# Denizantip/py-numpy-renderer

Hardware: AMD Instinct MI355X
Metric: Mfrag/s (1920x1080, 200k tris + shadow volumes) (higher is better)
Workload: dtype f64; 1 GPU; torus 500x200 (200k tris) + floor, 1920x1080, point light, shadow volumes (BASELINE.json configs[3] / BASELINE.md c4); faces=200002, views=8, frames_in_flight=3, parallelism=screen tiles x1 (bands)

## Files before the change

include/mi355rast.h:

```cpp
#ifndef MI355RAST_H
#define MI355RAST_H

#include <stdint.h>

#ifdef __cplusplus
extern "C" {
#endif

#define MR_ABI_VERSION 4

enum {
    MR_OK = 0,
    MR_E_INVALID = -1,
    MR_E_DEVICE = -2,
    MR_E_UNSUPPORTED = -3,
    MR_E_OVERFLOW = -4
};

enum { MR_LIGHT_DIRECTIONAL = 0, MR_LIGHT_POINT = 1, MR_LIGHT_SPOT = 2 };

enum {
    MR_FACE_RENDERED = 0, MR_FACE_BACK_FACE_CULLING = 1, MR_FACE_WRONG_MIN_MAX = 2,
    MR_FACE_EMPTY_B = 4, MR_FACE_EMPTY_Z = 8, MR_FACE_CLIPPED = 16
};
// ... 137 lines not shown
void mr_host_camera_constants(const double *eye, const double *center, const double *up, const double *position,
                              const double *projection, int32_t lh, double *lookat, double *mvp, double *planes);

int mr_host_overlay_build(const double *corners, const double *planes, const double *mvp, const double *viewport,
                          double near_plane, double far_plane, int32_t camera_inside, int32_t height, int32_t width,
                          int32_t *n_segments, int32_t *n_points, int32_t *n_touched);
int mr_host_overlay_fetch(int32_t *seg_first, int32_t *seg_count, int32_t *target, int32_t *next, double *z,
                          int32_t *touched);

int mr_render_device(mr_scene *scene, const mr_frame_desc *frame, void *d_out_rgb, void *stream);

int mr_get_stats(mr_scene *scene, mr_stats *stats);

#define MR_N_KERNEL_TIMES 5
int mr_get_kernel_times(mr_scene *scene, int n_frames, float *out_ms, int cap);
int mr_get_stream_kernel_times(mr_scene *scene, void *stream, int n_frames, float *out_ms, int cap);

int mr_read_z(mr_scene *scene, double *out_hw);
int mr_read_stencil(mr_scene *scene, int16_t *out_hw);
int mr_read_winner(mr_scene *scene, int32_t *out_hw);
int mr_read_frame_f32(mr_scene *scene, float *out_hw3);
int mr_read_face_status(mr_scene *scene, uint8_t *out_faces);
int mr_read_silhouette(mr_scene *scene, int32_t *out_triples, int32_t cap);
int mr_read_stencil_light(mr_scene *scene, int32_t light, int16_t *out_hw);
int mr_read_silhouette_light(mr_scene *scene, int32_t light, int32_t *out_triples, int32_t cap);

#define MR_TILE_RECORD_WORDS 12
int mr_debug_read_tile_records(mr_scene *scene, uint32_t *out, int32_t cap_tiles);

int mr_debug_clusters_culled(mr_scene *scene);

int mr_debug_quad_walks(mr_scene *scene, uint32_t *out);

int mr_debug_force_full(mr_scene *scene, int32_t on);

int mr_debug_frame_path(mr_scene *scene, int32_t *out);

int mr_debug_sil_cache(mr_scene *scene, int32_t *out);

int mr_debug_read_tile_order(mr_scene *scene, uint32_t *out, int32_t cap_tiles);

int mr_scene_set_model_pose(mr_scene *scene, int32_t model, const double *m16);

int mr_scene_set_model_pose_normals(mr_scene *scene, int32_t model, const double *g9);

int mr_debug_pose(mr_scene *scene, int32_t *out);

#define MR_N_POSE_TIMES 5
int mr_debug_pose_times(mr_scene *scene, float *out_ms);

#define MR_N_POSE_NORMALS_TIMES 2
int mr_debug_pose_normals_times(mr_scene *scene, float *out_ms);

int mr_scene_set_model_skin(mr_scene *scene, int32_t model, const int32_t *joints, const double *weights, int32_t n_bones,
                            const int32_t *normal_owner);

int mr_scene_set_model_bones(mr_scene *scene, int32_t model, const double *bones16, int32_t n_bones);

void mr_host_skin_chain(const double *verts, const int32_t *joints, const double *weights, const double *bones, int32_t n, double *out);

void mr_host_skin_chain3(const double *vectors, const int32_t *owner, const int32_t *joints, const double *weights, const double *bones,
                         int32_t n, double *out);

int mr_debug_skin(mr_scene *scene, int32_t *out);

#define MR_N_SKIN_TIMES 2
// ... 34 lines not shown
```

py-numpy-renderer_amd/_native.py:

```python
import ctypes as C
import os
import zlib

import numpy as np

from ._pack import active_morph, active_skin, auto_normals_active, morph_csr, normal_owners, pack_frame, pack_model, pose_normal_matrix

_HERE = os.path.dirname(os.path.abspath(__file__))
LIB_NAME = "libmi355rast.so"
LIB_PATH = os.path.join(_HERE, LIB_NAME)

MR_OK = 0
MR_E_OVERFLOW = -4
FRAME_SHADOWS, FRAME_KEEP_FLOAT, FRAME_FACE_STATUS, FRAME_LIGHT_TIMING, FRAME_SKYBOX, FRAME_COUNTERS = 1, 2, 4, 8, 16, 32
FRAME_KEEP_BUFFERS = 64
FRAME_NO_TIMING = 128
FRAME_OVERLAY = 256
FRAME_SUPERSAMPLE2, FRAME_SUPERSAMPLE4 = 512, 1024
_SUPERSAMPLE_FLAGS = {1: 0, 2: FRAME_SUPERSAMPLE2, 4: FRAME_SUPERSAMPLE4}
ABI_VERSION = 4
MAX_LIGHTS = 4
TILE_RECORD_WORDS = 12


# ... 72 lines not shown
    "mr_scene_add_model": (C.c_int, [C.c_void_p, C.POINTER(ModelDesc)]),
    "mr_scene_clear": (C.c_int, [C.c_void_p]),
    "mr_scene_set_overlay": (C.c_int, [C.c_void_p, C.POINTER(OverlayDesc)]),
    "mr_scene_set_overlay_cameras": (C.c_int, [C.c_void_p, C.c_void_p, C.c_void_p, C.c_void_p, C.c_void_p, C.c_double, C.c_double,
                                               C.c_int32, C.c_int32, C.c_int32]),
    "mr_scene_set_list_capacities": (C.c_int, [C.c_void_p, C.c_uint32, C.c_uint32, C.c_uint32, C.c_uint32]),
    "mr_scene_set_extra_lights": (C.c_int, [C.c_void_p, C.c_void_p, C.c_int32]),
    "mr_read_stencil_light": (C.c_int, [C.c_void_p, C.c_int32, C.c_void_p]),
    "mr_read_silhouette_light": (C.c_int, [C.c_void_p, C.c_int32, C.c_void_p, C.c_int32]),
    "mr_render": (C.c_int, [C.c_void_p, C.POINTER(FrameDesc), C.c_void_p, C.POINTER(Stats)]),
    "mr_overlay_state_bytes": (C.c_int64, [C.c_void_p]),
    "mr_overlay_apply": (C.c_int, [C.c_void_p, C.c_void_p, C.c_int64, C.c_int64, C.c_int32, C.c_int32, C.c_int32, C.c_void_p, C.c_void_p]),
    "mr_render_async": (C.c_int, [C.c_void_p, C.POINTER(FrameDesc), C.c_void_p, C.c_int32]),
    "mr_render_wait": (C.c_int, [C.c_void_p, C.c_int32, C.POINTER(Stats)]),
    "mr_host_alloc": (C.c_void_p, [C.c_uint64]),
    "mr_host_free": (None, [C.c_void_p]),
    "mr_render_device": (C.c_int, [C.c_void_p, C.POINTER(FrameDesc), C.c_void_p, C.c_void_p]),
    "mr_get_stats": (C.c_int, [C.c_void_p, C.POINTER(Stats)]),
    "mr_get_kernel_times": (C.c_int, [C.c_void_p, C.c_int, C.POINTER(C.c_float), C.c_int]),
    "mr_get_stream_kernel_times": (C.c_int, [C.c_void_p, C.c_void_p, C.c_int, C.POINTER(C.c_float), C.c_int]),
    "mr_read_z": (C.c_int, [C.c_void_p, C.c_void_p]),
    "mr_read_stencil": (C.c_int, [C.c_void_p, C.c_void_p]),
    "mr_read_winner": (C.c_int, [C.c_void_p, C.c_void_p]),
    "mr_read_frame_f32": (C.c_int, [C.c_void_p, C.c_void_p]),
    "mr_read_face_status": (C.c_int, [C.c_void_p, C.c_void_p]),
    "mr_read_silhouette": (C.c_int, [C.c_void_p, C.c_void_p, C.c_int32]),
    "mr_host_matmul_chain": (None, [C.c_void_p, C.c_void_p, C.c_void_p, C.c_int32, C.c_int32, C.c_int32]),
    "mr_host_overlay_build": (C.c_int, [C.c_void_p, C.c_void_p, C.c_void_p, C.c_void_p, C.c_double, C.c_double, C.c_int32,
                                        C.c_int32, C.c_int32, C.c_void_p, C.c_void_p, C.c_void_p]),
    "mr_host_overlay_fetch": (C.c_int, [C.c_void_p, C.c_void_p, C.c_void_p, C.c_void_p, C.c_void_p, C.c_void_p]),
    "mr_debug_read_tile_records": (C.c_int, [C.c_void_p, C.c_void_p, C.c_int32]),
    "mr_debug_clusters_culled": (C.c_int, [C.c_void_p]),
    "mr_debug_quad_walks": (C.c_int, [C.c_void_p, C.c_void_p]),
    "mr_host_camera_constants": (None, [C.c_void_p] * 5 + [C.c_int32] + [C.c_void_p] * 3),
    "mr_debug_read_tile_order": (C.c_int, [C.c_void_p, C.c_void_p, C.c_int32]),
    "mr_debug_sil_cache": (C.c_int, [C.c_void_p, C.c_void_p]),
    "mr_debug_force_full": (C.c_int, [C.c_void_p, C.c_int32]),
    "mr_debug_frame_path": (C.c_int, [C.c_void_p, C.c_void_p]),
    "mr_scene_set_model_pose": (C.c_int, [C.c_void_p, C.c_int32, C.c_void_p]),
    "mr_scene_set_model_pose_normals": (C.c_int, [C.c_void_p, C.c_int32, C.c_void_p]),
    "mr_debug_pose_normals_times": (C.c_int, [C.c_void_p, C.POINTER(C.c_float)]),
    "mr_debug_pose": (C.c_int, [C.c_void_p, C.c_void_p]),
    "mr_debug_pose_times": (C.c_int, [C.c_void_p, C.POINTER(C.c_float)]),
    "mr_debug_read_clusters": (C.c_int, [C.c_void_p, C.c_void_p, C.c_int32]),
    "mr_scene_set_model_skin": (C.c_int, [C.c_void_p, C.c_int32, C.c_void_p, C.c_void_p, C.c_int32, C.c_void_p]),
    "mr_scene_set_model_bones": (C.c_int, [C.c_void_p, C.c_int32, C.c_void_p, C.c_int32]),
    "mr_host_skin_chain": (None, [C.c_void_p, C.c_void_p, C.c_void_p, C.c_void_p, C.c_int32, C.c_void_p]),
    "mr_host_skin_chain3": (None, [C.c_void_p, C.c_void_p, C.c_void_p, C.c_void_p, C.c_void_p, C.c_int32, C.c_void_p]),
    "mr_debug_skin": (C.c_int, [C.c_void_p, C.c_void_p]),
    "mr_debug_skin_times": (C.c_int, [C.c_void_p, C.POINTER(C.c_float)]),
    "mr_scene_set_model_morph": (C.c_int, [C.c_void_p, C.c_int32, C.c_int32] + [C.c_void_p] * 6),
    "mr_scene_set_model_morph_weights": (C.c_int, [C.c_void_p, C.c_int32, C.c_void_p, C.c_int32]),
    "mr_host_morph_chain": (C.c_int, [C.c_void_p, C.c_int32, C.c_int32, C.c_int32] + [C.c_void_p] * 5),
    "mr_debug_morph": (C.c_int, [C.c_void_p, C.c_void_p]),
    "mr_debug_morph_times": (C.c_int, [C.c_void_p, C.POINTER(C.c_float)]),
    "mr_scene_set_model_auto_normals": (C.c_int, [C.c_void_p, C.c_int32, C.c_int32]),
    "mr_host_auto_normals": (C.c_int, [C.c_void_p, C.c_int32, C.c_void_p, C.c_int32, C.c_void_p, C.c_int32, C.c_void_p]),
    "mr_debug_auto_normals": (C.c_int, [C.c_void_p, C.c_void_p]),
    "mr_debug_auto_normals_times": (C.c_int, [C.c_void_p, C.POINTER(C.c_float)]),
    "mr_last_error": (C.c_char_p, []),
}
EXPORTED_SYMBOLS = tuple(_PROTOTYPES)

_lib = None


# ... 489 lines not shown
        _check(fn(self.handle, out.ctypes.data), fn.__name__)
        return out

    def read_z(self):
        return self._tap(self.lib.mr_read_z, np.float64)

    def read_stencil(self, light=0):
        h, w = self._frame
        out = np.empty((h, w), dtype=np.int16)
        _check(self.lib.mr_read_stencil_light(self.handle, int(light), out.ctypes.data), "mr_read_stencil_light")
        return out

    def read_winner(self):
        return self._tap(self.lib.mr_read_winner, np.int32)

    def read_frame_f32(self):
        return self._tap(self.lib.mr_read_frame_f32, np.float32, (3,))

    def read_tile_records(self):
        n = _check(self.lib.mr_debug_read_tile_records(self.handle, (C.c_uint32 * TILE_RECORD_WORDS)(), 0),
                   "mr_debug_read_tile_records")
        out = np.empty((max(n, 1), TILE_RECORD_WORDS), dtype=np.uint32)
        _check(self.lib.mr_debug_read_tile_records(self.handle, out.ctypes.data, n), "mr_debug_read_tile_records")
        return out[:n]

    def clusters_culled(self):
        return int(_check(self.lib.mr_debug_clusters_culled(self.handle), "mr_debug_clusters_culled"))

    def quad_walks(self):
        out = (C.c_uint32 * 4)()
        _check(self.lib.mr_debug_quad_walks(self.handle, out), "mr_debug_quad_walks")
        return tuple(int(x) for x in out)

    def sil_cache(self):
        out = (C.c_int32 * 4)()
        _check(self.lib.mr_debug_sil_cache(self.handle, out), "mr_debug_sil_cache")
        return tuple(int(x) for x in out)

    def force_full(self, on=True):
        _check(self.lib.mr_debug_force_full(self.handle, 1 if on else 0), "mr_debug_force_full")

    def frame_path(self):
        out = (C.c_int32 * 5)()
        _check(self.lib.mr_debug_frame_path(self.handle, out), "mr_debug_frame_path")
        return dict(zip(("full", "split", "ss", "ml", "ordered"), (bool(x) for x in out)))

    def pose_counters(self):
        out = (C.c_int32 * 4)()
        _check(self.lib.mr_debug_pose(self.handle, out), "mr_debug_pose")
        return tuple(int(x) for x in out)

    def skin_counters(self):
        out = (C.c_int32 * 4)()
        _check(self.lib.mr_debug_skin(self.handle, out), "mr_debug_skin")
        return tuple(int(x) for x in out)

    def morph_counters(self):
        out = (C.c_int32 * 5)()
        _check(self.lib.mr_debug_morph(self.handle, out), "mr_debug_morph")
        return tuple(int(x) for x in out)

    def auto_normals_counters(self):
        out = (C.c_int32 * 4)()
        _check(self.lib.mr_debug_auto_normals(self.handle, out), "mr_debug_auto_normals")
        return tuple(int(x) for x in out)

# ... 72 lines not shown
```

py-numpy-renderer_amd/csrc/host_env.h:

```cpp
#pragma once

namespace {

struct Env {
    bool vertex_mfma, resolve_separate, sil_cache;
    int edge_spread, tile_split, tile_order;
    int quad_walk;
    unsigned split_cost, split_quads;
    const char *cluster_cull;
};

Env read_env()
{
    static const Env once = [] {
        auto is = [](const char *name, const char *value) { const char *e = getenv(name); return e && !strcmp(e, value); };
        auto number = [](const char *name, int unset) { const char *e = getenv(name); return e ? atoi(e) : unset; };
        Env e = {};
        e.vertex_mfma = is("MR_VERTEX_PATH", "mfma");
        e.resolve_separate = is("MR_RESOLVE_PATH", "separate");
        e.edge_spread = number("MR_EDGE_SPREAD", -2);
        e.tile_order = is("MR_TILE_ORDER", "rowmajor") ? 1 : is("MR_TILE_ORDER", "heaviest") ? 2 : 0;
        e.quad_walk = is("MR_QUAD_WALK", "strips") ? 1 : is("MR_QUAD_WALK", "spans") ? 2 : 0;
        e.tile_split = number("MR_TILE_SPLIT", -1);
        e.split_cost = (unsigned)number("MR_SPLIT_COST", 400);
        e.split_quads = (unsigned)number("MR_SPLIT_QUADS", 48);
        return e;
    }();
    Env e = once;
    e.cluster_cull = getenv("MR_CLUSTER_CULL");
    const char *sil = getenv("MR_SIL_CACHE");
    e.sil_cache = !(sil && !strcmp(sil, "0"));
    return e;
}

}
```

py-numpy-renderer_amd/csrc/host_frame.h:

```cpp
#pragma once

namespace {

constexpr int EVENT_RING = 512, N_MARKS = 6;

struct FrameSlot {
    hipStream_t stream = nullptr;
    int id = 0;
    DevBuf d_vout, d_vclip, d_tris, d_clips, d_status, d_count_list, d_quads, d_sil, d_counters;
    DevBuf d_bin_count, d_items[mr::BIN_CLASSES], d_work, d_tile_stats, d_hist, d_split;
    DevBuf d_z, d_winner, d_stencil, d_frame, d_out;
    DevBuf d_stencil_x[mr::MAX_LIGHTS - 1];
    static_assert(mr::MAX_LIGHTS == MR_MAX_LIGHTS, "the ABI's light count is the kernels'");
    int last_n_lights = 1;
    uint32_t bin_cap[mr::BIN_CLASSES] = { 0, 0, 0 }, work_cap = 0, quad_cap = 0;
    int bins_zeroed_for = 0;

    mr::Counters *h_counters = nullptr;
    mr::Sticky *h_sticky = nullptr;
    hipEvent_t ev_ring[EVENT_RING][N_MARKS] = {};
    uint8_t ev_marks[EVENT_RING] = {};
    hipEvent_t *ev = ev_ring[0];
    uint64_t frames_enqueued = 0;
    uint64_t last_serial = 0;
// ... 403 lines not shown
        { { k_setup<true, true>, k_setup<false, true> }, { k_setup<true, false>, k_setup<false, false> } },
        { { k_setup_full<true, true>, k_setup_full<false, true> }, { k_setup_full<true, false>, k_setup_full<false, false> } } };
    hipLaunchKernelGGL(kernel[p.full][!p.ml][!p.env.vertex_mfma], dim3(1 + p.face_blocks + edge_blocks), dim3(SETUP_BLOCK), 0, stream, ska);
    return ska.sil.mode == SIL_CAPTURE ? sc->sil.capture_launched(&sa.ctr->n_quads, stream) : MR_OK;
}

void launch_bin_work(FrameSlot *fs, const mr::FrameConst &fc, const FramePlan &p)
{
    using namespace mr;
    hipLaunchKernelGGL(k_bin_work, dim3(p.count_blocks + WORK_BLOCKS), dim3(256), 0, fs->stream, fc, bin_args(fs), fs->d_count_list.as<uint32_t>(),
                       fs->d_tris.as<TriRec>(), fs->d_clips.as<TriClip>(), fs->d_status.as<uint8_t>(), fs->ctr(fs->frames_enqueued), p.count_blocks);
}

int launch_tile(mr_scene *sc, FrameSlot *fs, const mr::FrameConst &fc, const FramePlan &p, const mr::FrameLights &lights, uint8_t *d_out)
{
    using namespace mr;
    TileKernArgs tka;
    tka.fc = fc;
    TileArgs &ta = tka.ta;
    ta.clips = fs->d_clips.as<TriClip>(); ta.quads = fs->d_quads.as<QuadRec>();
    ta.bin_count = fs->d_bin_count.as<uint32_t>();
    for (int c = 0; c < BIN_CLASSES; ++c) { ta.items[c] = fs->d_items[c].as<uint32_t>(); ta.cap[c] = fs->bin_cap[c]; }
    ta.tap_mask = (p.overlay && !p.taps_asked) ? fs->ov.list<uint8_t>(3) : nullptr;
    ta.zbuf = p.keep ? fs->d_z.as<double>() : nullptr;
    ta.winner = p.keep ? fs->d_winner.as<int32_t>() : nullptr;
    ta.stencil = p.keep ? fs->d_stencil.as<int32_t>() : nullptr;
    ta.tile_stats = fs->d_tile_stats.as<uint32_t>();
    ta.ctr = fs->ctr(fs->frames_enqueued); ta.next_ctr = fs->ctr(fs->frames_enqueued + 1); ta.sticky = fs->sticky();
    ta.order = p.ordered ? fs->d_hist.as<uint32_t>() : nullptr;
    ta.tile_class = reinterpret_cast<uint8_t *>(fs->d_hist.p) + p.order_bytes;
    ta.split_arrive = fs->d_split.as<uint32_t>(); ta.split_sten = fs->d_split.as<int32_t>() + HEAVY0_MAX;
    ta.split_cost = p.split_cost; ta.split_quads = p.split_quads; ta.split_max = p.split_max;
    ta.quad_walk = (uint32_t)p.env.quad_walk;
    ShadeArgs &sh = tka.sh;
    sh.tris = fs->d_tris.as<TriRec>(); sh.face_pos = sc->d_face_pos.p; sh.face_attr = sc->d_face_attr.as<FaceAttr>();
    sh.materials = sc->d_materials.as<Material>();
    sh.sky = sc->sky_size > 0 ? sc->d_sky.as<uint8_t>() : nullptr;
    sh.gamma_lut = sc->d_gamma.as<float>(); sh.out = d_out;
    sh.frame = (fc.flags & MR_FRAME_KEEP_FLOAT) ? fs->d_frame.as<float>() : nullptr;
    tka.ml.lights.n = 1;
    if (p.ml) tka.ml.lights = lights;
    for (int k = 1; p.ml && k < MAX_LIGHTS; ++k) tka.ml.stencil[k - 1] = p.keep && k < p.n_lights ? fs->d_stencil_x[k - 1].as<int32_t>() : nullptr;
    if (p.n_tiles <= 0) {
        HIP_TRY(hipMemsetAsync(ta.next_ctr, 0, sizeof(Counters), fs->stream));
        return MR_OK;
    }
    static const struct { void (*kernel)(const TileKernArgs); int front; } choice[2][6] = {
        { { k_tile<false, true, true>, 0 },            { k_tile<false, false, true>, 0 },
          { k_tile<true, true, false>, SPLIT_FRONT },  { k_tile<true, false, false>, SPLIT_FRONT },
          { k_tile<false, true, false>, 0 },           { k_tile<false, false, false>, 0 } },
        { { k_tile_full<false, true, true>, 0 },           { k_tile_full<false, false, true>, 0 },
          { k_tile_full<true, true, false>, SPLIT_FRONT }, { k_tile_full<true, false, false>, SPLIT_FRONT },
          { k_tile_full<false, true, false>, 0 },          { k_tile_full<false, false, false>, 0 } } };
    const auto &c = choice[p.full][(p.ml ? 0 : p.split ? 2 : 4) + !p.ss];
    hipLaunchKernelGGL(c.kernel, dim3((unsigned)(p.n_tiles + c.front)), dim3(TILE_PX), 0, fs->stream, tka);
    return MR_OK;
}

void launch_after_tile(mr_scene *sc, FrameSlot *fs, const mr_frame_desc *fr, const mr::FrameConst &fc, const FramePlan &p, uint8_t *d_out)
{
    using namespace mr;
    hipStream_t stream = fs->stream;
    if ((fc.flags & MR_FRAME_FACE_STATUS) && fc.n_faces > 0)
        hipLaunchKernelGGL(k_face_status, dim3(blocks_for(fc.n_faces, 256)), dim3(256), 0, stream, fc, fs->d_tris.as<TriRec>(),
                           fs->d_clips.as<TriClip>(), fs->d_z.as<double>(), fs->d_stencil.as<int32_t>(), fs->d_status.as<uint8_t>());
    if (p.overlay && p.partial) {
// ... 156 lines not shown
```

py-numpy-renderer_amd/csrc/kernels_tile.h:

```cpp
#pragma once

#include "kernels_bin.h"
#include "kernels_shade.h"

namespace mr {

__device__ __forceinline__ unsigned long long z_key(double z)
{
    const unsigned long long b = (unsigned long long)__double_as_longlong(z);
    return (b >> 63) ? ~b : (b | 0x8000000000000000ull);
}
__device__ __forceinline__ double z_unkey(unsigned long long k)
{
    const unsigned long long b = (k >> 63) ? (k & 0x7fffffffffffffffull) : ~k;
    return __longlong_as_double((long long)b);
}

template <bool MAYBE_SINGLE>
struct PairMath {
    double a0, a1, p0, p1, q0, q1, k0, k1, k2;
    float d00, d01, d11, inv_den;
    bool sbox, sz;
    __device__ __forceinline__ explicit PairMath(const TriRec &t)
    {
// ... 7 lines not shown
    }
    __device__ __forceinline__ void bary(double x, double y, float &u, float &v, float &w) const
    {
        const double r0 = (sbox ? x : y) - a0, r1 = (sbox ? y : x) - a1;
        const float d20 = (float)fma(r1, p1, r0 * p0);
        const float d21 = (float)fma(r1, q1, r0 * q0);
        v = (d11 * d20 - d01 * d21) * inv_den;
        w = (d00 * d21 - d01 * d20) * inv_den;
        u = 1.0f - v - w;
    }
    __device__ __forceinline__ void bary(int x, int y, float &u, float &v, float &w) const
    {
        bary((double)(sbox ? x : y), (double)(sbox ? y : x), true, u, v, w);
    }
    __device__ __forceinline__ double depth(float u, float v, float w) const
    {
        const float m0 = sz ? u : v, m1 = sz ? v : u;
        return fma((double)w, k2, fma((double)m1, k1, (double)m0 * k0));
    }
private:
    __device__ __forceinline__ void bary(double c0, double c1, bool, float &u, float &v, float &w) const
    {
        const double r0 = c0 - a0, r1 = c1 - a1;
        const float d20 = (float)fma(r1, p1, r0 * p0);
        const float d21 = (float)fma(r1, q1, r0 * q0);
        v = (d11 * d20 - d01 * d21) * inv_den;
        w = (d00 * d21 - d01 * d20) * inv_den;
        u = 1.0f - v - w;
    }
};

constexpr int SMALL_LANES = 4;

constexpr int SWEEP_CACHE_K = 2, SWEEP_CACHE_ROUNDS = 2;
struct SweepCache {
    unsigned long long key[SWEEP_CACHE_K];
    uint32_t meta;
};

struct TileBounds { int width, band_y0, band_y1; };

template <int SWEEP, bool FULL>
__device__ __forceinline__ void small_pair(const TileBounds &tb, const TriRec &t, int gx, int gy, bool rh,
                                           unsigned long long *s_key, int *s_win, int sub, int lanes, unsigned int &frags,
                                           SweepCache *cache = nullptr, int first = 0)
{
    const int x0 = max((int)t.x0, gx), x1 = min((int)t.x1, min(gx + TILE_W, tb.width));
    const int y0 = max(max((int)t.y0, gy), tb.band_y0), y1 = min(min((int)t.y1, gy + TILE_H), tb.band_y1);
    const PairMath<true> pm(t);
    const bool nodepth = FULL && ((t.flags >> 8) & FF_NO_DEPTH) != 0;
    const int bw = x1 - x0;
    if (cache) { cache->meta = 0; }
    if (bw <= 0) return;
    int px = x0 + sub, py = y0;
    while (px >= x1) { px -= bw; ++py; }
    int walked = 0;
    while (py < y1) {
        if (SWEEP == 0 || walked >= first) {
            float u, v, w;
            pm.bary(px, py, u, v, w);
            bool ok = u >= 0 && v >= 0 && w >= 0;
            if (FULL && ok && SWEEP == 0) ++frags;
            if (ok && (SWEEP == 1 || !nodepth)) {
                const double z = pm.depth(u, v, w);
                if (z == z) {
                    const int p = (py - gy) * TILE_W + (px - gx);
                    const unsigned long long k = z_key(z);
                    if (SWEEP == 0) {
                        if (rh) atomicMin(&s_key[p], k); else atomicMax(&s_key[p], k);
                        if (cache) {
#pragma unroll
                            for (int c = 0; c < SWEEP_CACHE_K; ++c)
                                if (walked == c) { cache->key[c] = k; cache->meta |= ((uint32_t)p << (8 * c)) | (1u << (16 + c)); }
                        }
                    } else if (nodepth ? (rh ? k <= s_key[p] : k >= s_key[p]) : s_key[p] == k) {
                        atomicMax(&s_win[p], t.face);
                    }
                }
            }
        }
        ++walked;
        px += lanes;
        while (px >= x1) { px -= bw; ++py; }
    }
    if (cache) cache->meta |= (uint32_t)walked << 20;
}

__device__ __forceinline__ int out_row(const FrameConst &fc, int py, int l)
{
    if (fc.out_tile_rows > 0)
        return (fc.out_tile_rows - 1 - l) * TILE_H + (tile_row_frame(fc, l) * TILE_H + TILE_H - 1 - py);
    return fc.band_y1 - 1 - py;
}

__device__ __forceinline__ uint8_t *ss_out_pixel(uint8_t *out, int width, int band_y1, int shift, int px, int py)
{
    return out + ((size_t)((band_y1 - 1 - py) >> shift) * (width >> shift) + (px >> shift)) * 3;
}
__device__ __forceinline__ void ss_block_mean(const float *rgb, int row, int shift, float m[3])
{
    const int s = 1 << shift;
    float acc[3] = { 0.f, 0.f, 0.f };
    for (int j = 0; j < s; ++j)
        for (int i = 0; i < s; ++i) {
#pragma unroll
            for (int c = 0; c < 3; ++c) acc[c] += rgb[j * row + i * 3 + c];
        }
    const float inv = 1.0f / (float)(s * s);
#pragma unroll
    for (int c = 0; c < 3; ++c) m[c] = acc[c] * inv;
}
__device__ __forceinline__ void ss_resolve_tile(const FrameConst &fc, const float *s_rgb, uint8_t *out, int gx, int gy, int tid,
                                                const float *s_gamma)
{
    const int shift = fc.ss_mode & SS_SHIFT_MASK, n_log = 4 - shift;
    static_assert(TILE_W == 16 && TILE_H == 16, "ss_resolve_tile");
    if (tid >= 1 << (2 * n_log)) return;
    const int bx = tid & ((1 << n_log) - 1), by = tid >> n_log;
// ... 55 lines not shown
#define MR_CLASS_SCALE 100
#endif
__device__ __forceinline__ int tile_class(uint32_t cost)
{
    const uint32_t c = cost * 100u / (uint32_t)MR_CLASS_SCALE;
    return c >= 500u ? 1 : c >= 350u ? 2 : c >= 250u ? 3 : c >= 170u ? 4 : c >= 110u ? 5 : c >= 70u ? 6 : c >= 40u ? 7 : 8;
}
static_assert(ORDER_CLASSES == 8, "tile_class");
#ifndef MR_HEAVY0_MAX
#define MR_HEAVY0_MAX 128
#endif
constexpr int HEAVY_SPLIT = 4, HEAVY0_MAX = MR_HEAVY0_MAX;
#ifndef MR_TILE_WAVES
#define MR_TILE_WAVES 5
#endif
constexpr int K_TILE_WAVES = MR_TILE_WAVES;
#ifndef MR_TILE_WAVES_1L
#define MR_TILE_WAVES_1L 6
#endif
constexpr int K_TILE_WAVES_1L = MR_TILE_WAVES_1L;
constexpr int SPLIT_FRONT = HEAVY_SPLIT * HEAVY0_MAX;

__device__ __forceinline__ uint32_t tile_cost(uint32_t n_small, uint32_t n_big, uint32_t n_quad)
{
    return 20u + 2u * n_small + 30u * n_big + 3u * n_quad;
}

struct TileArgs {
    const TriClip *clips;
    const QuadRec *quads;
    uint32_t *bin_count;
    const uint32_t *items[BIN_CLASSES];
    uint32_t cap[BIN_CLASSES];
    const uint8_t *tap_mask;
    double *zbuf;
    int32_t *winner, *stencil;
    uint32_t *tile_stats;
    Counters *ctr, *next_ctr;
    Sticky *sticky;
    int32_t *split_sten;
    uint32_t *split_arrive;
    const uint32_t *order;
    uint8_t *tile_class;
    uint32_t split_cost, split_quads;
    uint32_t split_max;
    uint32_t quad_walk;
};

struct TileLights {
    FrameLights lights;
    int32_t *stencil[MAX_LIGHTS - 1];
};
struct TileKernArgs { FrameConst fc; TileArgs ta; ShadeArgs sh; TileLights ml; };

template <bool SPLIT, bool SS, bool ML, bool FULL>
__device__ __forceinline__ void tile_body()
{
    static_assert(!(SPLIT && ML), "frames with several lights do not split their heavy tiles");
    __shared__ unsigned long long s_key[TILE_PX];
    __shared__ int s_win[TILE_PX];
    __shared__ unsigned int s_cnt[TILE_STATS];
    __shared__ uint4 s_quad[QUAD_BATCH * QUAD_STAGE_U4];
    __shared__ uint32_t s_id[QUAD_BATCH];
    __shared__ float s_gamma[GAMMA_LUT_SIZE];
    __shared__ unsigned long long s_mat[MAT_LDS * sizeof(Material) / 8];

// ... 77 lines not shown
                if (ss) {
                    float *s_rgb = reinterpret_cast<float *>(s_quad);
#pragma unroll
                    for (int j = 0; j < 3; ++j) s_rgb[lp * 3 + j] = rgb[j];
                }
                __syncthreads();
                if (ss) {
                    ss_resolve_tile(fc, reinterpret_cast<const float *>(s_quad), sh.out, gx, gy, tid, s_gamma);
                } else if (live) {
#pragma unroll
                    for (int j = 0; j < 3; ++j) o[j] = gamma_u8(rgb[j], s_gamma);
                }
            } else if (ss) {
                const int shift = ss & SS_SHIFT_MASK, n_log = 4 - shift;
                const int bpx = gx + ((tid & ((1 << n_log) - 1)) << shift), bpy = gy + ((tid >> n_log) << shift);
                if (tid < 1 << (2 * n_log) && bpx < fc.width && bpy >= fc.band_y0 && bpy < fc.band_y1) {
                    uint8_t *ob = ss_out_pixel(sh.out, fc.width, fc.band_y1, shift, bpx, bpy);
                    ob[0] = (uint8_t)fc.background_u8; ob[1] = (uint8_t)(fc.background_u8 >> 8); ob[2] = (uint8_t)(fc.background_u8 >> 16);
                }
            } else if (live) {
                o[0] = (uint8_t)fc.background_u8; o[1] = (uint8_t)(fc.background_u8 >> 8); o[2] = (uint8_t)(fc.background_u8 >> 16);
            }
            if (tid == 0) {
                uint32_t *rec = ta.tile_stats + (size_t)tile * TILE_REC;
                for (int k = 0; k < TILE_REC; ++k) rec[k] = 0;
                rec[7] = n_quad_raw;
                rec[8] = rec[10] = rec[11] = (uint32_t)t_start;
                rec[9] = (uint32_t)stamp();
                ta.bin_count[2 * n_tiles + tile] = 0;
                ta.tile_class[tile] = (uint8_t)ORDER_CLASSES;
            }
            return;
        }
        if (FULL && tid < TILE_STATS) s_cnt[tid] = 0;
        s_gamma[tid] = sh.gamma_lut[tid];
        if (tid == 0) s_gamma[GAMMA_LUT_SIZE - 1] = sh.gamma_lut[GAMMA_LUT_SIZE - 1];
        mat_lds = fc.n_materials <= MAT_LDS;
        if (mat_lds && tid < fc.n_materials * (int)(sizeof(Material) / 8))
            s_mat[tid] = reinterpret_cast<const unsigned long long *>(sh.materials)[tid];
    }
    auto my_pixel = [&](int &px, int &py) {
        int l = lp;
        asm volatile("" : "+v"(l));
        px = gx + (l & (TILE_W - 1)); py = gy + l / TILE_W;
    };

    double zbest = rh ? INFINITY : -INFINITY;
    int best = -1;
    {
        const TileKernArgs &ka = kernargs<TileKernArgs>();
        const FrameConst &fc = ka.fc;
        const TileArgs &ta = ka.ta;
        const ShadeArgs &sh = ka.sh;
        const TriRec *__restrict__ tris = sh.tris;
        const TriClip *__restrict__ clips = ta.clips;
        const uint32_t *__restrict__ small_items = ta.items[0] + (size_t)tile * ta.cap[0];
        const uint32_t *__restrict__ big_items = ta.items[1] + (size_t)tile * ta.cap[1];
        const bool same_clip = fc.same_clip != 0, has_no_depth = FULL && fc.has_no_depth != 0;
        const TileBounds tb = { fc.width, fc.band_y0, fc.band_y1 };
        int px, py;
        my_pixel(px, py);
        const double dpx = (double)px, dpy = (double)py;
        unsigned int frags = 0;
        constexpr int TRI_U4 = (int)(sizeof(TriRec) / 16);
        static_assert(WAVE * TRI_U4 <= QUAD_BATCH * QUAD_STAGE_U4, "big-pair records are staged in the quad area");
        auto big_pairs = [&](const bool late) {
// ... 17 lines not shown
                        float u, v, w;
                        pm.bary(dpx, dpy, u, v, w);
                        in = in && u >= 0 && v >= 0 && w >= 0;
                        const unsigned long long m = __ballot(in);
                        if (!m) return;
                        if (FULL && !late) frags += (unsigned int)__popcll(m);
                        if (nodepth && !late) return;
                        if (flags & TF_CLIP) {
                            if (in) {
                                const TriClip &c = clips[f];
                                double p[3];
                                persp_bary(t.dp, u, v, w, (flags & TF_SINGLE_BOX) != 0, p);
                                in = inside_clip(p, c.clip) && (same_clip || inside_clip(p, c.clipd));
                            }
                        }
                        const double z = pm.depth(u, v, w);
                        if (late) {
                            if (in && (rh ? z <= zbest : z >= zbest) && f > best) best = f;
                        } else {
                            const bool closer = rh ? (z < zbest) : (z > zbest);
                            if (in && (closer || (z == zbest && f > best))) { zbest = z; best = f; }
                        }
                    };
                    if (flags & (TF_SINGLE_BOX | TF_SINGLE_Z)) pair(std::true_type{});
                    else pair(std::false_type{});
                }
            }
        };
        big_pairs(false);
        if (n_small) { s_key[lp] = z_key(zbest); s_win[lp] = -1; }
        __syncthreads();
        if (FULL && lane == 0 && frags) atomicAdd(&s_cnt[0], frags);
        if (n_small) {
            unsigned long long (*c_key)[SWEEP_CACHE_K][TILE_PX] =
                reinterpret_cast<unsigned long long (*)[SWEEP_CACHE_K][TILE_PX]>(s_quad);
            uint32_t (*c_meta)[TILE_PX] = reinterpret_cast<uint32_t (*)[TILE_PX]>(
                reinterpret_cast<unsigned long long *>(s_quad) + SWEEP_CACHE_ROUNDS * SWEEP_CACHE_K * TILE_PX);
            uint32_t (*c_face)[TILE_PX] = c_meta + SWEEP_CACHE_ROUNDS;
            static_assert(SWEEP_CACHE_ROUNDS * TILE_PX * (SWEEP_CACHE_K * 8 + 8) <= (int)sizeof(s_quad), "sweep cache fits the quad area");
            unsigned int sfrags = 0;
            int round = 0;
            const int spl = n_small > (uint32_t)(TILE_PX / SMALL_LANES) ? SMALL_LANES / 2
                          : n_small > (uint32_t)(TILE_PX / (2 * SMALL_LANES)) ? SMALL_LANES : 2 * SMALL_LANES;
            const uint32_t per_round = (uint32_t)(TILE_PX / spl), my_pair = (uint32_t)(tid / spl);
            const int sub = tid % spl;
            for (uint32_t i = my_pair; i < n_small; i += per_round, ++round) {
                const TriRec t = tris[small_items[i]];
                if (round < SWEEP_CACHE_ROUNDS) {
                    SweepCache sc;
                    small_pair<0, FULL>(tb, t, gx, gy, rh, s_key, s_win, sub, spl, sfrags, &sc);
                    const bool nodepth = FULL && ((t.flags >> 8) & FF_NO_DEPTH) != 0;
#pragma unroll
                    for (int c = 0; c < SWEEP_CACHE_K; ++c) c_key[round][c][tid] = sc.key[c];
                    c_meta[round][tid] = nodepth ? (sc.meta & 0xfff00000u) : sc.meta;
                    c_face[round][tid] = (uint32_t)t.face | (nodepth ? 0x80000000u : 0u);
                } else {
                    small_pair<0, FULL>(tb, t, gx, gy, rh, s_key, s_win, sub, spl, sfrags);
                }
            }
            if (FULL && sfrags) atomicAdd(&s_cnt[0], sfrags);
            __syncthreads();

            const unsigned long long kfinal = s_key[lp];
            if (best >= 0 && kfinal == z_key(zbest)) atomicMax(&s_win[lp], best);
            round = 0;
            for (uint32_t i = my_pair; i < n_small; i += per_round, ++round) {
                int first = 0;
                if (round < SWEEP_CACHE_ROUNDS) {
                    const uint32_t meta = c_meta[round][tid], cf = c_face[round][tid];
                    const int walked = (int)(meta >> 20);
                    const bool nodepth = FULL && (cf >> 31) != 0;
#pragma unroll
                    for (int c = 0; c < SWEEP_CACHE_K; ++c)
                        if ((meta >> (16 + c)) & 1u) {
                            const int p = (int)((meta >> (8 * c)) & 0xffu);
                            if (s_key[p] == c_key[round][c][tid]) atomicMax(&s_win[p], (int)(cf & 0x7fffffffu));
                        }
                    if (!nodepth && walked <= SWEEP_CACHE_K) continue;
                    first = nodepth ? 0 : SWEEP_CACHE_K;
                }
                const TriRec t = tris[small_items[i]];
                small_pair<1, FULL>(tb, t, gx, gy, rh, s_key, s_win, sub, spl, sfrags, nullptr, first);
            }
            __syncthreads();
            best = s_win[lp];
            zbest = z_unkey(kfinal);
        }
        if (has_no_depth) big_pairs(true);
    }
    const bool covered = live && best >= 0;
    const unsigned long long t_raster = stamp();

    int sten = 0;
    int sten_x[MAX_LIGHTS - 1] = { 0, 0, 0 };
    unsigned int qfrags = 0, qupd = 0;
    if (n_quad && (counters || __syncthreads_or(covered))) {
        const TileKernArgs &ka = kernargs<TileKernArgs>();
        const FrameConst &fc = ka.fc;
        const TileArgs &ta = ka.ta;
        const uint32_t *__restrict__ quad_items = ta.items[2] + (size_t)tile * ta.cap[2];
        const QuadRec *__restrict__ quads = ta.quads;
        const double f_plus_n = fc.f_plus_n, f_minus_n = fc.f_minus_n, two_nf = fc.two_nf;
        double zlim = rh ? -INFINITY : INFINITY, zhard = rh ? INFINITY : -INFINITY;
        if (covered) zlim = zhard = zbest;
#pragma unroll
        for (int off = WAVE / 2; off; off >>= 1) {
            const double o = __shfl_xor(zlim, off), h = __shfl_xor(zhard, off);
            zlim = rh ? fmax(zlim, o) : fmin(zlim, o);
            zhard = rh ? fmin(zhard, h) : fmax(zhard, h);
        }
        if (!FULL) {
            zlim = __hiloint2double(__builtin_amdgcn_readfirstlane(__double2hiint(zlim)), __builtin_amdgcn_readfirstlane(__double2loint(zlim)));
            zhard = __hiloint2double(__builtin_amdgcn_readfirstlane(__double2hiint(zhard)), __builtin_amdgcn_readfirstlane(__double2loint(zhard)));
        }
        if (!ML && ta.quad_walk != QUAD_WALK_STRIPS) {
// ... 331 lines not shown
            ta.zbuf[at_px] = zbest;
            ta.winner[at_px] = best;
            ta.stencil[at_px] = sten;
        }
    }
    static_assert(TILE_PX * 3 * sizeof(float) <= sizeof(s_quad), "resolve staging fits the quad area");
    if (fused_ss) {
        __syncthreads();
        const TileKernArgs &ka = kernargs<TileKernArgs>();
        ss_resolve_tile(ka.fc, reinterpret_cast<const float *>(s_quad), ka.sh.out, gx, gy, tid, s_gamma);
    }

    if (counters) {
        const unsigned long long cov = __ballot(covered), litm = __ballot(covered && lit);
        if (ML) {
            unsigned int v = covered ? n_lit : 0u;
#pragma unroll
            for (int off = WAVE / 2; off; off >>= 1) v += (unsigned int)__shfl_xor((int)v, off);
            if (lane == 0 && v) atomicAdd(&s_cnt[4], v);
        }
        if (lane == 0) {
            if (cov) atomicAdd(&s_cnt[3], (unsigned int)__popcll(cov));
            if (!ML && litm) atomicAdd(&s_cnt[4], (unsigned int)__popcll(litm));
            if (qfrags) atomicAdd(&s_cnt[1], qfrags);
            if (qupd) atomicAdd(&s_cnt[2], qupd);
        }
    }
    if (FULL) __syncthreads();
    const TileArgs &ta = kernargs<TileKernArgs>().ta;
    uint32_t *rec = ta.tile_stats + (size_t)tile * TILE_REC;
    if (FULL && tid < TILE_STATS) rec[tid] = s_cnt[tid];
    if (tid == 0) {
        rec[5] = n_small_raw; rec[6] = n_big_raw; rec[7] = n_quad_raw;
        rec[8] = (uint32_t)t_start;
        rec[9] = (uint32_t)stamp();
        rec[10] = (uint32_t)t_raster; rec[11] = (uint32_t)t_quads;
        if (n_small_raw > ta.cap[0]) { atomicOr(&ta.ctr->overflow, 1u); atomicMax(&ta.ctr->max_list[0], n_small_raw); }
        if (n_big_raw > ta.cap[1]) { atomicOr(&ta.ctr->overflow, 2u); atomicMax(&ta.ctr->max_list[1], n_big_raw); }
        if (n_quad_raw > ta.cap[2]) { atomicOr(&ta.ctr->overflow, 4u); atomicMax(&ta.ctr->max_list[2], n_quad_raw); }
    }
    if (tid < BIN_CLASSES) ta.bin_count[tid * n_tiles + tile] = 0;
    if (tid == 0) {
        int cls = tile_class(cost);
        if (SPLIT) cls = (cost >= ta.split_cost && n_quad_raw >= ta.split_quads) ? 1 : cls < 2 ? 2 : cls;
        ta.tile_class[tile] = (uint8_t)cls;
    }
}

template <bool SPLIT, bool SS, bool ML>
__global__ void __launch_bounds__(TILE_PX, ML ? K_TILE_WAVES : K_TILE_WAVES_1L)
k_tile(const TileKernArgs)
{
    tile_body<SPLIT, SS, ML, false>();
}
template <bool SPLIT, bool SS, bool ML>
__global__ void __launch_bounds__(TILE_PX, ML ? K_TILE_WAVES : K_TILE_WAVES_1L)
k_tile_full(const TileKernArgs)
{
    tile_body<SPLIT, SS, ML, true>();
}

__global__ void __launch_bounds__(256)
k_reduce_tile_stats(const uint32_t *__restrict__ tile_stats, int n_tiles, Counters *__restrict__ ctr, int counted)
{
    constexpr int NS = TILE_STATS + 2;
    __shared__ unsigned long long part[NS][256 / WAVE];
    const int tid = threadIdx.x, lane = tid & (WAVE - 1), wv = tid / WAVE;
// ... 62 lines not shown
```

py-numpy-renderer_amd/csrc/mi355rast.hip:

```cpp
#include "../../include/mi355rast.h"
#include "host_overlay.h"

#include <hip/hip_runtime.h>

#include <algorithm>
#include <array>
#include <cmath>
#include <cstdio>
#include <cstdlib>
#include <cstring>
#include <memory>
#include <new>
#include <string>
#include <vector>

#include "rast_types.h"
#include "kernels_geometry.h"
#include "kernels_tile.h"
#include "kernels_overlay.h"
#include "kernels_pose.h"

#include "host_device.h"
#include "host_env.h"
#include "host_silcache.h"
// ... 757 lines not shown
    if (!out) return fail(MR_E_INVALID, "NULL argument");
    const int n = std::min(fs->last_n_tiles, cap_tiles);
    HIP_TRY(hipDeviceSynchronize());
    static_assert(mr::TILE_REC == MR_TILE_RECORD_WORDS, "tile record size is part of the ABI");
    if (n > 0) HIP_TRY(hipMemcpy(out, fs->d_tile_stats.p, (size_t)n * mr::TILE_REC * 4, hipMemcpyDeviceToHost));
    if (!fs->last_full)
        for (int t = 0; t < n; ++t)
            for (int k = 0; k < mr::TILE_STATS; ++k) out[(size_t)t * mr::TILE_REC + k] = 0u;
    return fs->last_n_tiles;
}

int mr_debug_clusters_culled(mr_scene *sc)
{
    FrameSlot *fs = last_slot(sc);
    if (!fs) return MR_E_INVALID;
    HIP_TRY(hipDeviceSynchronize());
    if (int rc = fetch_counters(fs, false)) return rc;
    HIP_TRY(hipStreamSynchronize(fs->stream));
    return (int)fs->h_counters->pad0[0];
}

int mr_debug_quad_walks(mr_scene *sc, uint32_t *out)
{
    FrameSlot *fs = last_slot(sc);
    if (!fs) return MR_E_INVALID;
    if (!out) return fail(MR_E_INVALID, "NULL argument");
    HIP_TRY(hipDeviceSynchronize());
    if (int rc = fetch_counters(fs, false)) return rc;
    HIP_TRY(hipStreamSynchronize(fs->stream));
    for (int k = 0; k < 4; ++k) out[k] = fs->h_counters->pad0[1 + k];
    return MR_OK;
}

int mr_debug_force_full(mr_scene *sc, int32_t on)
{
    if (!sc) return fail(MR_E_INVALID, "NULL argument");
    sc->force_full = on != 0;
    return MR_OK;
}

int mr_debug_frame_path(mr_scene *sc, int32_t *out)
{
    FrameSlot *fs = last_slot(sc);
    if (!fs) return MR_E_INVALID;
    if (!out) return fail(MR_E_INVALID, "NULL argument");
    out[0] = fs->last_full ? 1 : 0; out[1] = fs->last_split ? 1 : 0; out[2] = fs->last_ss_mode ? 1 : 0;
    out[3] = fs->last_n_lights > 1 ? 1 : 0; out[4] = fs->last_ordered ? 1 : 0;
    return MR_OK;
}

int mr_debug_sil_cache(mr_scene *sc, int32_t *out)
{
    if (!sc || !out) return fail(MR_E_INVALID, "NULL argument");
    out[0] = sc->sil.last_path; out[1] = (int32_t)sc->sil.last_entries; out[2] = (int32_t)sc->sil.captures;
    out[3] = sc->sil.valid_buffers();
    return MR_OK;
}

int mr_debug_pose(mr_scene *sc, int32_t *out)
{
    if (!sc || !out) return fail(MR_E_INVALID, "NULL argument");
    int32_t posed = 0;
    for (const mr_scene::ModelPose &mp : sc->poses) posed += mp.posed ? 1 : 0;
    out[0] = sc->commits; out[1] = sc->pose_passes; out[2] = posed; out[3] = sc->pose_written;
    return MR_OK;
}
// ... 132 lines not shown
```

Baseline: 37790 Mfrag/s.

## Replace per-round sweep cache with a per-thread pair log and resume point

```diff
diff --git a/include/mi355rast.h b/include/mi355rast.h
--- a/include/mi355rast.h
+++ b/include/mi355rast.h
@@ -193,6 +193,8 @@
 
 int mr_debug_quad_walks(mr_scene *scene, uint32_t *out);
 
+int mr_debug_pair_log(mr_scene *scene, uint32_t *out);
+
 int mr_debug_force_full(mr_scene *scene, int32_t on);
 
 int mr_debug_frame_path(mr_scene *scene, int32_t *out);
diff --git a/py-numpy-renderer_amd/_native.py b/py-numpy-renderer_amd/_native.py
--- a/py-numpy-renderer_amd/_native.py
+++ b/py-numpy-renderer_amd/_native.py
@@ -128,6 +128,7 @@
     "mr_debug_read_tile_records": (C.c_int, [C.c_void_p, C.c_void_p, C.c_int32]),
     "mr_debug_clusters_culled": (C.c_int, [C.c_void_p]),
     "mr_debug_quad_walks": (C.c_int, [C.c_void_p, C.c_void_p]),
+    "mr_debug_pair_log": (C.c_int, [C.c_void_p, C.c_void_p]),
     "mr_host_camera_constants": (None, [C.c_void_p] * 5 + [C.c_int32] + [C.c_void_p] * 3),
     "mr_debug_read_tile_order": (C.c_int, [C.c_void_p, C.c_void_p, C.c_int32]),
     "mr_debug_sil_cache": (C.c_int, [C.c_void_p, C.c_void_p]),
@@ -683,6 +684,11 @@
         _check(self.lib.mr_debug_quad_walks(self.handle, out), "mr_debug_quad_walks")
         return tuple(int(x) for x in out)
 
+    def pair_log(self):
+        out = (C.c_uint32 * 2)()
+        _check(self.lib.mr_debug_pair_log(self.handle, out), "mr_debug_pair_log")
+        return tuple(int(x) for x in out)
+
     def sil_cache(self):
         out = (C.c_int32 * 4)()
         _check(self.lib.mr_debug_sil_cache(self.handle, out), "mr_debug_sil_cache")
diff --git a/py-numpy-renderer_amd/csrc/host_env.h b/py-numpy-renderer_amd/csrc/host_env.h
--- a/py-numpy-renderer_amd/csrc/host_env.h
+++ b/py-numpy-renderer_amd/csrc/host_env.h
@@ -6,6 +6,7 @@
     bool vertex_mfma, resolve_separate, sil_cache;
     int edge_spread, tile_split, tile_order;
     int quad_walk;
+    int pair_log;
     unsigned split_cost, split_quads;
     const char *cluster_cull;
 };
@@ -21,6 +22,7 @@
         e.edge_spread = number("MR_EDGE_SPREAD", -2);
         e.tile_order = is("MR_TILE_ORDER", "rowmajor") ? 1 : is("MR_TILE_ORDER", "heaviest") ? 2 : 0;
         e.quad_walk = is("MR_QUAD_WALK", "strips") ? 1 : is("MR_QUAD_WALK", "spans") ? 2 : 0;
+        e.pair_log = std::min(std::max(number("MR_PAIR_LOG", mr::PAIR_LOG_K), 0), (int)mr::PAIR_LOG_K);
         e.tile_split = number("MR_TILE_SPLIT", -1);
         e.split_cost = (unsigned)number("MR_SPLIT_COST", 400);
         e.split_quads = (unsigned)number("MR_SPLIT_QUADS", 48);
diff --git a/py-numpy-renderer_amd/csrc/host_frame.h b/py-numpy-renderer_amd/csrc/host_frame.h
--- a/py-numpy-renderer_amd/csrc/host_frame.h
+++ b/py-numpy-renderer_amd/csrc/host_frame.h
@@ -459,6 +459,7 @@
     ta.split_arrive = fs->d_split.as<uint32_t>(); ta.split_sten = fs->d_split.as<int32_t>() + HEAVY0_MAX;
     ta.split_cost = p.split_cost; ta.split_quads = p.split_quads; ta.split_max = p.split_max;
     ta.quad_walk = (uint32_t)p.env.quad_walk;
+    ta.pair_log = (uint32_t)fc.n_faces <= PAIR_LOG_MAX_FACE ? (uint32_t)p.env.pair_log : 0u;
     ShadeArgs &sh = tka.sh;
     sh.tris = fs->d_tris.as<TriRec>(); sh.face_pos = sc->d_face_pos.p; sh.face_attr = sc->d_face_attr.as<FaceAttr>();
     sh.materials = sc->d_materials.as<Material>();
diff --git a/py-numpy-renderer_amd/csrc/kernels_tile.h b/py-numpy-renderer_amd/csrc/kernels_tile.h
--- a/py-numpy-renderer_amd/csrc/kernels_tile.h
+++ b/py-numpy-renderer_amd/csrc/kernels_tile.h
@@ -63,26 +63,30 @@
 
 constexpr int SMALL_LANES = 4;
 
-constexpr int SWEEP_CACHE_K = 2, SWEEP_CACHE_ROUNDS = 2;
-struct SweepCache {
-    unsigned long long key[SWEEP_CACHE_K];
-    uint32_t meta;
+constexpr int PAIR_LOG_K = 4;
+constexpr uint32_t PAIR_LOG_NONE = 0xffffffffu, PAIR_LOG_MAX_FACE = 1u << 24;
+struct PairLog {
+    unsigned long long (*key)[TILE_PX];
+    uint32_t (*word)[TILE_PX];
+    uint32_t n, cap;
+    uint32_t resume;
 };
 
 struct TileBounds { int width, band_y0, band_y1; };
 
-template <int SWEEP, bool FULL>
-__device__ __forceinline__ void small_pair(const TileBounds &tb, const TriRec &t, int gx, int gy, bool rh,
+template <int SWEEP, bool FULL, bool COUNT = FULL>
+__device__ __forceinline__ uint32_t small_pair(const TileBounds &tb, const TriRec &t, int gx, int gy, bool rh,
                                            unsigned long long *s_key, int *s_win, int sub, int lanes, unsigned int &frags,
-                                           SweepCache *cache = nullptr, int first = 0)
+                                           PairLog *log = nullptr, int tid = 0, int first = 0)
 {
     const int x0 = max((int)t.x0, gx), x1 = min((int)t.x1, min(gx + TILE_W, tb.width));
     const int y0 = max(max((int)t.y0, gy), tb.band_y0), y1 = min(min((int)t.y1, gy + TILE_H), tb.band_y1);
     const PairMath<true> pm(t);
     const bool nodepth = FULL && ((t.flags >> 8) & FF_NO_DEPTH) != 0;
     const int bw = x1 - x0;
-    if (cache) { cache->meta = 0; }
-    if (bw <= 0) return;
+    uint32_t over = PAIR_LOG_NONE;
+    if (SWEEP == 0 && nodepth) { log->cap = 0; over = 0; }
+    if (bw <= 0) return over;
     int px = x0 + sub, py = y0;
     while (px >= x1) { px -= bw; ++py; }
     int walked = 0;
@@ -91,7 +95,7 @@
             float u, v, w;
             pm.bary(px, py, u, v, w);
             bool ok = u >= 0 && v >= 0 && w >= 0;
-            if (FULL && ok && SWEEP == 0) ++frags;
+            if (COUNT) frags += SWEEP == 0 ? (ok ? 1u : 0u) : 1u;
             if (ok && (SWEEP == 1 || !nodepth)) {
                 const double z = pm.depth(u, v, w);
                 if (z == z) {
@@ -99,10 +103,11 @@
                     const unsigned long long k = z_key(z);
                     if (SWEEP == 0) {
                         if (rh) atomicMin(&s_key[p], k); else atomicMax(&s_key[p], k);
-                        if (cache) {
-#pragma unroll
-                            for (int c = 0; c < SWEEP_CACHE_K; ++c)
-                                if (walked == c) { cache->key[c] = k; cache->meta |= ((uint32_t)p << (8 * c)) | (1u << (16 + c)); }
+                        const bool fits = log->n < log->cap;
+                        over = fits ? over : min(over, (uint32_t)walked);
+                        if (fits) {
+                            log->key[log->n][tid] = k; log->word[log->n][tid] = (uint32_t)p | ((uint32_t)t.face << 8);
+                            ++log->n;
                         }
                     } else if (nodepth ? (rh ? k <= s_key[p] : k >= s_key[p]) : s_key[p] == k) {
                         atomicMax(&s_win[p], t.face);
@@ -114,7 +119,7 @@
         px += lanes;
         while (px >= x1) { px -= bw; ++py; }
     }
-    if (cache) cache->meta |= (uint32_t)walked << 20;
+    return over;
 }
 
 __device__ __forceinline__ int out_row(const FrameConst &fc, int py, int l)
@@ -236,6 +241,7 @@
     uint32_t *bin_count;
     const uint32_t *items[BIN_CLASSES];
     uint32_t cap[BIN_CLASSES];
+    uint32_t pair_log;
     const uint8_t *tap_mask;
     double *zbuf;
     int32_t *winner, *stencil;
@@ -379,6 +385,7 @@
             }
             return;
         }
+        if (FULL && tid == 0) ta.tile_stats[(size_t)tile * TILE_REC + 8] = (uint32_t)t_start;
         if (FULL && tid < TILE_STATS) s_cnt[tid] = 0;
         s_gamma[tid] = sh.gamma_lut[tid];
         if (tid == 0) s_gamma[GAMMA_LUT_SIZE - 1] = sh.gamma_lut[GAMMA_LUT_SIZE - 1];
@@ -462,55 +469,50 @@
         __syncthreads();
         if (FULL && lane == 0 && frags) atomicAdd(&s_cnt[0], frags);
         if (n_small) {
-            unsigned long long (*c_key)[SWEEP_CACHE_K][TILE_PX] =
-                reinterpret_cast<unsigned long long (*)[SWEEP_CACHE_K][TILE_PX]>(s_quad);
-            uint32_t (*c_meta)[TILE_PX] = reinterpret_cast<uint32_t (*)[TILE_PX]>(
-                reinterpret_cast<unsigned long long *>(s_quad) + SWEEP_CACHE_ROUNDS * SWEEP_CACHE_K * TILE_PX);
-            uint32_t (*c_face)[TILE_PX] = c_meta + SWEEP_CACHE_ROUNDS;
-            static_assert(SWEEP_CACHE_ROUNDS * TILE_PX * (SWEEP_CACHE_K * 8 + 8) <= (int)sizeof(s_quad), "sweep cache fits the quad area");
+            static_assert(PAIR_LOG_K * TILE_PX * (8 + 4) <= (int)sizeof(s_quad), "the pair log fits the quad area");
+            PairLog log;
+            log.key = reinterpret_cast<unsigned long long (*)[TILE_PX]>(s_quad);
+            log.word = reinterpret_cast<uint32_t (*)[TILE_PX]>(log.key + PAIR_LOG_K);
+            log.n = 0;
+            log.cap = FULL && ML ? 0u : min(kernargs<TileKernArgs>().ta.pair_log, (uint32_t)PAIR_LOG_K);
+            log.resume = log.cap ? PAIR_LOG_NONE : 0u;
             unsigned int sfrags = 0;
-            int round = 0;
             const int spl = n_small > (uint32_t)(TILE_PX / SMALL_LANES) ? SMALL_LANES / 2
                           : n_small > (uint32_t)(TILE_PX / (2 * SMALL_LANES)) ? SMALL_LANES : 2 * SMALL_LANES;
             const uint32_t per_round = (uint32_t)(TILE_PX / spl), my_pair = (uint32_t)(tid / spl);
             const int sub = tid % spl;
-            for (uint32_t i = my_pair; i < n_small; i += per_round, ++round) {
+            for (uint32_t i = my_pair; i < n_small; i += per_round) {
                 const TriRec t = tris[small_items[i]];
-                if (round < SWEEP_CACHE_ROUNDS) {
-                    SweepCache sc;
-                    small_pair<0, FULL>(tb, t, gx, gy, rh, s_key, s_win, sub, spl, sfrags, &sc);
-                    const bool nodepth = FULL && ((t.flags >> 8) & FF_NO_DEPTH) != 0;
-#pragma unroll
-                    for (int c = 0; c < SWEEP_CACHE_K; ++c) c_key[round][c][tid] = sc.key[c];
-                    c_meta[round][tid] = nodepth ? (sc.meta & 0xfff00000u) : sc.meta;
-                    c_face[round][tid] = (uint32_t)t.face | (nodepth ? 0x80000000u : 0u);
-                } else {
-                    small_pair<0, FULL>(tb, t, gx, gy, rh, s_key, s_win, sub, spl, sfrags);
-                }
+                const uint32_t over = small_pair<0, FULL>(tb, t, gx, gy, rh, s_key, s_win, sub, spl, sfrags, &log, tid);
+                log.resume = (log.resume == PAIR_LOG_NONE && over != PAIR_LOG_NONE) ? ((i / per_round) << 8) | over : log.resume;
             }
             if (FULL && sfrags) atomicAdd(&s_cnt[0], sfrags);
             __syncthreads();
 
             const unsigned long long kfinal = s_key[lp];
             if (best >= 0 && kfinal == z_key(zbest)) atomicMax(&s_win[lp], best);
-            round = 0;
-            for (uint32_t i = my_pair; i < n_small; i += per_round, ++round) {
-                int first = 0;
-                if (round < SWEEP_CACHE_ROUNDS) {
-                    const uint32_t meta = c_meta[round][tid], cf = c_face[round][tid];
-                    const int walked = (int)(meta >> 20);
-                    const bool nodepth = FULL && (cf >> 31) != 0;
-#pragma unroll
-                    for (int c = 0; c < SWEEP_CACHE_K; ++c)
-                        if ((meta >> (16 + c)) & 1u) {
-                            const int p = (int)((meta >> (8 * c)) & 0xffu);
-                            if (s_key[p] == c_key[round][c][tid]) atomicMax(&s_win[p], (int)(cf & 0x7fffffffu));
-                        }
-                    if (!nodepth && walked <= SWEEP_CACHE_K) continue;
-                    first = nodepth ? 0 : SWEEP_CACHE_K;
-                }
-                const TriRec t = tris[small_items[i]];
-                small_pair<1, FULL>(tb, t, gx, gy, rh, s_key, s_win, sub, spl, sfrags, nullptr, first);
+            const uint32_t n_logged = log.n;
+#pragma unroll
+            for (uint32_t e = 0; e < (uint32_t)PAIR_LOG_K; ++e)
+                if (e < n_logged) {
+                    const uint32_t w = log.word[e][tid], p = w & 0xffu;
+                    if (s_key[p] == log.key[e][tid]) atomicMax(&s_win[p], (int)(w >> 8));
+                }
+            sfrags = 0;
+            if (log.resume != PAIR_LOG_NONE) {
+                int first = (int)(log.resume & 0xffu);
+                for (uint32_t i = my_pair + (log.resume >> 8) * per_round; i < n_small; i += per_round) {
+                    const TriRec t = tris[small_items[i]];
+                    small_pair<1, FULL, FULL>(tb, t, gx, gy, rh, s_key, s_win, sub, spl, sfrags, nullptr, tid, first);
+                    first = 0;
+                }
+            }
+            if (counters) {
+                unsigned int a = n_logged, b = sfrags;
+#pragma unroll
+                for (int off = WAVE / 2; off; off >>= 1) { a += __shfl_xor(a, off); b += __shfl_xor(b, off); }
+                if (lane == 0 && a) atomicAdd(&ta.ctr->pad0[5], a);
+                if (lane == 0 && b) atomicAdd(&ta.ctr->pad0[6], b);
             }
             __syncthreads();
             best = s_win[lp];
@@ -908,7 +910,7 @@
     if (FULL && tid < TILE_STATS) rec[tid] = s_cnt[tid];
     if (tid == 0) {
         rec[5] = n_small_raw; rec[6] = n_big_raw; rec[7] = n_quad_raw;
-        rec[8] = (uint32_t)t_start;
+        if (!FULL) rec[8] = 0;
         rec[9] = (uint32_t)stamp();
         rec[10] = (uint32_t)t_raster; rec[11] = (uint32_t)t_quads;
         if (n_small_raw > ta.cap[0]) { atomicOr(&ta.ctr->overflow, 1u); atomicMax(&ta.ctr->max_list[0], n_small_raw); }
diff --git a/py-numpy-renderer_amd/csrc/mi355rast.hip b/py-numpy-renderer_amd/csrc/mi355rast.hip
--- a/py-numpy-renderer_amd/csrc/mi355rast.hip
+++ b/py-numpy-renderer_amd/csrc/mi355rast.hip
@@ -813,6 +813,18 @@
     return MR_OK;
 }
 
+int mr_debug_pair_log(mr_scene *sc, uint32_t *out)
+{
+    FrameSlot *fs = last_slot(sc);
+    if (!fs) return MR_E_INVALID;
+    if (!out) return fail(MR_E_INVALID, "NULL argument");
+    HIP_TRY(hipDeviceSynchronize());
+    if (int rc = fetch_counters(fs, false)) return rc;
+    HIP_TRY(hipStreamSynchronize(fs->stream));
+    for (int k = 0; k < 2; ++k) out[k] = fs->h_counters->pad0[5 + k];
+    return MR_OK;
+}
+
 int mr_debug_force_full(mr_scene *sc, int32_t on)
 {
     if (!sc) return fail(MR_E_INVALID, "NULL argument");
```

New measurement: 38730 Mfrag/s, median of 6. 2.5% higher.
